# loehnea/bensolve

Measured on AMD Instinct MI355X. Metric: scalar LPs/sec (Benson phase 2, batched P2(v) solves incl. cut application), synthetic VLP q=5 n=500 m=1000, higher is better.
Workload: dtype f64

## Files before the change

### bensolve_amd/csrc/poly_engine.hip

```cpp
#include "common.h"
#include <vector>
#include <chrono>
#include <algorithm>
#include <cmath>
#include <thread>
#include <atomic>
#include <cstddef>

namespace bslv {

constexpr int MAXD = 16;
constexpr double POLY_EPS = 1e-9;
constexpr int PB = 256;
constexpr unsigned char F_USED = 1, F_IDEAL = 2, F_SLTN = 4;
constexpr int CRING = 1024;
constexpr int CSTRIDE = 8;
constexpr int LCAP = 16;
constexpr int LONGN = 64;
constexpr int ZMAX = 8;

struct Hp { double h[MAXD + 1]; };
struct Tri { int a, b, c; };

struct PolyView {
// ... 1965 lines not shown
        const int cv = __shfl(first, src, WAVE);
        const int *cL = D.fpool + D.foff[cj];
        const int cnj = D.flen[cj];
        const int *pool = P.pool + P.inc_off[cv];
        const int npool = P.inc_len[cv];
        bool found = false;
        for (int base = 0; base < npool; base += WAVE) {
            int k = base + lane;
            bool hit = false;
            if (k < npool) {
                int w = pool[k];
                if (w != fi && w != cj && D.flive[w] && D.flen[w] >= cn)
                    hit = isect3_count(A, ni, cL, cnj, D.fpool + D.foff[w], D.flen[w]) == cn;
            }
            if (__ballot(hit)) { found = true; break; }
        }
        if (lane == src) adj = !found;
    }
    Tri t{adj ? 1 : 0, 0, 0};
    pflag[(size_t)blockIdx.x * PB + threadIdx.x] = adj ? 1 : 0;
    Tri tot;
    (void)block_exscan(t, &tot, lds);
    if (threadIdx.x == 0) bsum[blockIdx.x] = tot;
}


__global__ __launch_bounds__(PB) void k_live_ranks(PolyView P, int nv, unsigned char *live)
{
    const int i = blockIdx.x * (PB / WAVE) + (threadIdx.x >> 6), lane = threadIdx.x & 63;
    if (i >= nv || !(P.flag[i] & F_USED)) return;
    const int *L = P.pool + P.inc_off[i];
    const int n = P.inc_len[i];
    for (int j = lane; j < n; j += WAVE) live[L[j]] = 1;
}
__global__ void k_bench_fill(PolyView P, int nv, unsigned long long seed)
{
    int i = blockIdx.x * blockDim.x + threadIdx.x;
    if (i >= nv) return;
    for (int k = 0; k < P.d; k++) {
        unsigned long long z = seed + 0x9E3779B97F4A7C15ull * ((unsigned long long)i * P.d + k + 1);
        z = (z ^ (z >> 30)) * 0xBF58476D1CE4E5B9ull;
        z = (z ^ (z >> 27)) * 0x94D049BB133111EBull;
        z ^= z >> 31;
        P.X[(size_t)k * P.cap + i] = (double)(z >> 11) * (1.0 / 9007199254740992.0) * 2.0 - 1.0;
    }
    P.flag[i] = F_USED;
    P.inc_len[i] = 0;
    P.inc_off[i] = 0;
}
#include "poly_rounds_kernels.inc"
#include "poly_rounds2_kernels.inc"
__device__ void k2v2_check_members(const K2V2 &V, int vs, const int *s_mem, int nm, const int *members, int nzero)
{
    RState *st = const_cast<RState *>(V.st);
    for (int m = threadIdx.x; m < nm; m += blockDim.x)
        for (int m2 = m + 1; m2 < nm; m2++)
            if (s_mem[m] == s_mem[m2] && atomicCAS(&st->err, 0, 4) == 0) {
                int c1 = -1, c2 = -1;
                for (int c = 0; c < nzero; c++) if (members[c] == s_mem[m]) { if (c1 < 0) c1 = c; else c2 = c; }
                st->err_info[0] = vs; st->err_info[1] = m; st->err_info[2] = m2; st->err_info[3] = s_mem[m]; st->err_info[4] = c1; st->err_info[5] = c2; st->err_info[6] = nzero;
            }
}
__device__ __forceinline__ int k2v2_round(const RState *st) { return st->round; }
__device__ __forceinline__ int k2v2_rank_base(const RState *st) { return st->rank_base; }
__device__ __forceinline__ void k2v2_sizes(const RState *st, int &S, int &go, int &nzero, int &nv0, int &ncross)
{
    S = st->S; go = st->go && !r2_halted(st); nzero = st->nzero; nv0 = st->nv; ncross = st->ncross;
}


}

using namespace bslv;

struct RoundsBuf;
struct Rounds2Buf;
struct bslv_poly {
    RoundsBuf *rounds = nullptr;
    Rounds2Buf *rounds2 = nullptr;
    bool rounds2_enabled = true;
    bool r2_spec = true;
    long r2_spec_void = 0;
    bool r2_mis = true;
    int chunk_cuts = 1024;
    int r2_defer = 0;
    bool r2_deferred = false;
    long r2_deferred_cuts = 0, r2_doomed = 0;
    bool r2_defer_mark = !(getenv("BSLV_DEFER_MARK") && atoi(getenv("BSLV_DEFER_MARK")) == 0);
    bool snap = false;
    unsigned long long *snapped_d = nullptr;
    int r2_min_cuts = 0;
    long r2_rounds = 0, r2_cuts = 0, r2_fallback_prunes = 0, r2_declined = 0, r2_chunks = 0, shuffle_seq = 0, r2_late_left = 0, r2_torn_reads = 0;
    long r2_fb_reason[5] = {0, 0, 0, 0, 0}, r2_fb_nm[20] = {0};
    int batch_mode = 1;
    long rounds_run = 0, conf_pairs = 0, conf_cuts = 0;
    int dense_streak = 0, dense_skip = 0;
    int d = 0, v2h = 0;
    std::vector<double> c;
    hipStream_t stream = nullptr;
    PolyView P{};
    int nv = 0;
    unsigned poolcap = 0, poolused = 0;
    int2 *E[2] = {nullptr, nullptr};
    int ecap = 0, ne = 0, ecur = 0;
    unsigned char *eflag = nullptr;
    int *ecount = nullptr; int ecountcap = 0;
    int *EP[2] = {nullptr, nullptr};
    bool hot = false, hot_enabled = true;
    struct EdgeSet { int2 *E[2] = {nullptr, nullptr}; int *EP[2] = {nullptr, nullptr}; unsigned char *eflag = nullptr; int ecap = 0, ne = 0, ecur = 0; } full, hotbuf;
    unsigned char *alive = nullptr; int alivecap = 0;
    int *hv_d = nullptr; int hvcap = 0;
    int *lslot_d = nullptr; int lslotcap = 0;
    unsigned *lbits_d = nullptr; size_t lbitscap = 0; int *lnslots_d = nullptr;
    long hot_chunks = 0, hot_elems = 0, hot_edges = 0;
    long n_spec = 0, n_declined = 0, n_k2_fallback = 0, n_single = 0;
    double tm_hot_begin = 0, tm_seq = 0, tm_hot_end = 0, tm_add_cuts = 0; long tm_seq_cuts = 0;
    double tm_realloc = 0; long n_realloc = 0;
    double tm_prep = 0, tm_classify_wait = 0, tm_newdual = 0;
    double tm_launch[4] = {0, 0, 0, 0};
    int *members = nullptr;
    Tri *bsum = nullptr; int bsumcap = 0;
    Tri *bsum2 = nullptr; size_t bsum2cap = 0;
    int *fm_cnt = nullptr, *fm_list = nullptr; size_t fmcap = 0, fmlistcap = 0; int fm_min = 4096; long n_fm = 0; bool member_lists = true;
    int largest_facet = 0;
    bool k2_noflags = getenv("BSLV_K2_NOFLAGS") != nullptr; long n_noflag_prunes = 0;
    long long window_blocks = 0x7FFFFFF0ll, win_max_blocks = 0; long n_win_prunes = 0, n_windows = 0;
    int shard_min = 32768; long n_sharded = 0; int2 *shard_e = nullptr; size_t shardcap = 0;
    int *nzlist = nullptr; size_t nzcap = 0;
    Tri *totals = nullptr;
    int *counters = nullptr;
    Tri *totals_h = nullptr; int *counters_h = nullptr;
    Mail *mail_h = nullptr, *mail_d = nullptr;
    Mail mail_v[4];
    long mail_torn_reads = 0;
    Mail *k2mail_d = nullptr;
    int *fstamp = nullptr, *flocal = nullptr, *nlocal = nullptr; int fcap = 0;
    unsigned long long *bits = nullptr; size_t bitscap = 0;
    int mailseq = 0;
    long cutseq = 0;
    size_t k2_lds = 0;
    int *ne_dev = nullptr;
    bool pend_k2 = false;
    int pend_seq = 0, pend_slot = 2, pend_ebase = 0, pend_nm = 0, pend_stamp = 0, pend_nzero = 0, pend_nv0 = 0, pend_ncross = 0; long long pend_len_ub = 0;
    int k2flip = 0;
    bool speculate = true;
    int cross_ub = CROSS_UB;
    CutDev *cutdev = nullptr;
    int *abort_d = nullptr;
    int *fcount = nullptr;
    int *zlist = nullptr, *zrows = nullptr;
    int pre_f = -1, pre_slot = 0, pre_nv = 0, pre_seq = 0;
    unsigned long long *k2dbg = nullptr;
    FILE *cutlog = nullptr;
    PairBlk *blks = nullptr; int blkcap = 0;
    unsigned char *pflag = nullptr; size_t pflagcap = 0;
    std::vector<double> Y, hp;
    std::vector<unsigned char> fapplied, fideal;
    std::vector<int> facet_of_rank;
    int nf = 0;
    bool initialised = false;
    std::vector<int> queue;
    std::vector<int> dual_edges;
    long pair_tests = 0, new_vertices = 0, cuts_applied = 0;
    double *hps_d = nullptr; int hpscap = 0; std::vector<double> hps_stage;
    unsigned long long *clsw = nullptr; size_t clswcap = 0;
    int *live_d = nullptr; int livecap = 0;
// ... 760 lines not shown
    for (int k = 0; k < d; k++)
        HIP_TRY(hipMemcpy(h->P.X + (size_t)k * h->P.cap, &soa[(size_t)k * n], n * sizeof(double), hipMemcpyHostToDevice));
    std::vector<unsigned char> fl(n, F_USED);
    for (int i = 1; i < n; i++) fl[i] |= F_IDEAL;
    HIP_TRY(hipMemcpy(h->P.flag, fl.data(), n, hipMemcpyHostToDevice));
    std::vector<unsigned> off(n);
    std::vector<int> len(n), pool;
    for (int i = 0; i < n; i++) { off[i] = (unsigned)pool.size(); len[i] = (int)inc[i].size(); pool.insert(pool.end(), inc[i].begin(), inc[i].end()); }
    HIP_TRY(hipMemcpy(h->P.inc_off, off.data(), n * sizeof(unsigned), hipMemcpyHostToDevice));
    HIP_TRY(hipMemcpy(h->P.inc_len, len.data(), n * sizeof(int), hipMemcpyHostToDevice));
    HIP_TRY(hipMemcpy(h->P.pool, pool.data(), pool.size() * sizeof(int), hipMemcpyHostToDevice));
    h->poolused = (unsigned)pool.size();
    std::vector<int2> E;
    for (int k = 0; k <= d; k++) for (int j = k + 1; j <= d; j++) E.push_back(int2{k, j});
    HIP_TRY(hipMemcpy(h->E[h->ecur], E.data(), E.size() * sizeof(int2), hipMemcpyHostToDevice));
    h->ne = (int)E.size();
    h->nv = n;
    h->facet_of_rank.resize(h->nf);
    for (int f = 0; f < h->nf; f++) h->facet_of_rank[f] = f;
    return 0;
}

static double gs_step(const double *x, double *H, double *R, int k, int n)
{
    double nrm_in = 0, scl = 0;
    for (int l = 0; l < n; l++) nrm_in += x[l] * x[l];
    nrm_in = std::sqrt(nrm_in);
    double *hr = H + (size_t)k * n;
    for (int l = 0; l < n; l++) hr[l] = x[l];
    for (int j = 0; j < k; j++) {
        double s = 0;
        for (int l = 0; l < n; l++) s += H[(size_t)j * n + l] * hr[l];
        for (int l = 0; l < n; l++) hr[l] -= s * H[(size_t)j * n + l];
    }
    for (int l = 0; l < n; l++) scl += hr[l] * hr[l];
    scl = std::sqrt(scl);
    if (scl < 1.0e-6) return 0;
    for (int l = 0; l < n; l++) hr[l] /= scl;
    for (int j = 0; j <= k; j++) {
        double s = 0;
        for (int l = 0; l < n; l++) s += H[(size_t)j * n + l] * x[l];
        R[k * (k + 1) / 2 + j] = s;
    }
    return scl / nrm_in;
}

extern "C" {

int bslv_poly_create(bslv_poly **out, int dim, int v2h, const double *c)
{
    if (!out || dim < 2 || dim > MAXD || v2h < 0 || v2h > 2) { set_error("bslv_poly_create: bad argument (2 <= dim <= %d)", MAXD); return BSLV_E_ARG; }
    if (bslv_device_count() < 1) { set_error("no HIP device available"); return BSLV_E_NODEVICE; }
    bslv_poly *h = new bslv_poly();
    h->d = dim; h->v2h = v2h;
    h->c.assign(dim, 0.0);
    if (c) h->c.assign(c, c + dim);
    h->P.d = dim;
    auto fail = [&](int code) { bslv_poly_destroy(h); return code; };
    if (hipStreamCreate(&h->stream) != hipSuccess) { set_error("hipStreamCreate failed"); return fail(BSLV_E_NODEVICE); }
    if (malloc0(&h->totals, 4 * sizeof(Tri)) != hipSuccess || malloc0(&h->counters, CRING * CSTRIDE * sizeof(int)) != hipSuccess || malloc0(&h->ne_dev, 4 * sizeof(int)) != hipSuccess || malloc0(&h->k2mail_d, 4 * sizeof(Mail)) != hipSuccess || hipMemset(h->k2mail_d, 0, 4 * sizeof(Mail)) != hipSuccess || malloc0(&h->cutdev, CRING * sizeof(CutDev)) != hipSuccess ||
        malloc0(&h->abort_d, 4 * sizeof(int)) != hipSuccess || hipMemset(h->abort_d, 0, 4 * sizeof(int)) != hipSuccess || malloc0(&h->zlist, CRING * ZMAX * sizeof(int)) != hipSuccess ||
        hipHostMalloc(&h->totals_h, 4 * sizeof(Tri)) != hipSuccess || hipHostMalloc(&h->counters_h, 4 * sizeof(int)) != hipSuccess ||
        hipHostMalloc(&h->mail_h, 4 * sizeof(Mail), hipHostMallocMapped | hipHostMallocCoherent) != hipSuccess ||
        hipHostGetDevicePointer((void **)&h->mail_d, h->mail_h, 0) != hipSuccess ||
        hipMemset(h->counters, 0, CRING * CSTRIDE * sizeof(int)) != hipSuccess) {
        set_error("allocation of scan scratch failed");
        return fail(BSLV_E_NOMEM);
    }
    memset((void *)h->mail_h, 0, 4 * sizeof(Mail));
    memset((void *)h->mail_v, 0, sizeof h->mail_v);
    for (int k = 0; k < 4; k++) h->mail_h[k].chk2 = mail_sum2(Tri{0, 0, 0}, 0);
    h->k2_lds = 128 * 1024;
    if (hipFuncSetAttribute((const void *)k2_fused_t<false>, hipFuncAttributeMaxDynamicSharedMemorySize, (int)h->k2_lds) != hipSuccess ||
        hipFuncSetAttribute((const void *)k2_fused_t<true>, hipFuncAttributeMaxDynamicSharedMemorySize, (int)h->k2_lds) != hipSuccess) {
        (void)hipGetLastError();
        h->k2_lds = 48 * 1024;
    }
    if (const char *cl = getenv("BSLV_CUT_LOG")) h->cutlog = fopen(cl, "w");
    if (getenv("BSLV_NO_SPEC")) h->speculate = false;
    if (getenv("BSLV_NO_HOT")) h->hot_enabled = false;
    if (getenv("BSLV_NO_ROUNDS2")) h->rounds2_enabled = false;
    if (const char *e = getenv("BSLV_R2_MIS")) h->r2_mis = atoi(e) != 0;
    if (const char *e = getenv("BSLV_R2_SPEC")) h->r2_spec = atoi(e) != 0;
    if (const char *e = getenv("BSLV_CHUNK_CUTS")) h->chunk_cuts = std::min(4096, std::max(32, atoi(e)));
    if (const char *e = getenv("BSLV_R2_MIN_CUTS")) h->r2_min_cuts = std::max(-1, atoi(e));
    if (const char *e = getenv("BSLV_POLY_SNAP")) h->snap = atoi(e) != 0;
    if (const char *e = getenv("BSLV_CROSS_UB")) h->cross_ub = std::max(0, atoi(e));
    if (const char *e = getenv("BSLV_K2_LDS")) h->k2_lds = (size_t)std::max(64, atoi(e));
    if (const char *e = getenv("BSLV_K2_WINDOW")) { const long long v = atoll(e); if (v > 0) h->window_blocks = std::min(v, PAIR_WINDOW_DEFAULT); }
    if (getenv("BSLV_K2_DEBUG") && malloc0(&h->k2dbg, 16 * sizeof(unsigned long long)) == hipSuccess) (void)hipMemset(h->k2dbg, 0, 16 * sizeof(unsigned long long));
    h->rounds = new RoundsBuf();
    std::vector<double> z(dim, 0.0);
    z[dim - 1] = -1.0;
    new_dual(h, z.data(), 1);
    *out = h;
    return 0;
}

void bslv_poly_destroy(bslv_poly *h)
{
    if (!h) return;
    if (getenv("BSLV_R2_REPORT") && h->r2_fallback_prunes) {
        fprintf(stderr, "r2: %ld prunes of rounds went through the multi-kernel path: %ld members > %d, %ld pair bitmap, %ld hash table, %ld bit matrix | members by power of two:", h->r2_fallback_prunes,
                h->r2_fb_reason[1], K2_MAXNM, h->r2_fb_reason[2], h->r2_fb_reason[3], h->r2_fb_reason[4]);
        for (int k = 0; k < 20; k++) if (h->r2_fb_nm[k]) fprintf(stderr, " 2^%d: %ld", k, h->r2_fb_nm[k]);
        fprintf(stderr, "\n");
    }
    if (getenv("BSLV_TIMING"))
        fprintf(stderr, "poly timing: add_cuts %.1f ms | hot_begin %.1f, sequences %.1f (%ld cuts, %.1f us each), hot_end %.1f ms | %ld hot chunks, %.0f elements, %.0f edges on average\n", h->tm_add_cuts,
                h->tm_hot_begin, h->tm_seq, h->tm_seq_cuts, h->tm_seq_cuts ? h->tm_seq * 1e3 / h->tm_seq_cuts : 0.0, h->tm_hot_end, h->hot_chunks,
                h->hot_chunks ? (double)h->hot_elems / h->hot_chunks : 0.0, h->hot_chunks ? (double)h->hot_edges / h->hot_chunks : 0.0),
        fprintf(stderr, "poly timing, per batch of cuts: dual slots %.2f ms, chunk preparation %.2f ms, waiting for the batched classification %.2f ms (totals); %ld re-allocations of element / edge / pool arrays, %.2f ms\n", h->tm_newdual, h->tm_prep, h->tm_classify_wait, h->n_realloc, h->tm_realloc),
        fprintf(stderr, "poly host per cut (us): queue round A %.1f, k_emit2 %.1f, round B in all %.1f, mailbox wait %.1f\n", h->tm_launch[0] / std::max(1L, h->n_single), h->tm_launch[1] / std::max(1L, h->n_single),
                h->tm_launch[2] / std::max(1L, h->n_single), h->tm_launch[3] / std::max(1L, h->n_single));
    if (h->cutlog) fclose(h->cutlog);
    if (h->k2dbg) {
        unsigned long long t[16];
        if (hipMemcpy(t, h->k2dbg, sizeof(t), hipMemcpyDeviceToHost) == hipSuccess && t[7])
            fprintf(stderr, "k2_fused phases (us/launch over %llu launches; rounds: per prune workgroup): P0a %.2f P0 %.2f P1 %.2f P2 %.2f P3 %.2f P4 %.2f P5 %.2f P6 %.2f | W %.1f nloc %.0f | members mean %.0f max %llu\n", t[7],
                    t[10] * 0.01 / t[7], t[0] * 0.01 / t[7], t[1] * 0.01 / t[7], t[2] * 0.01 / t[7], t[3] * 0.01 / t[7], t[4] * 0.01 / t[7], t[5] * 0.01 / t[7], t[6] * 0.01 / t[7], (double)t[8] / t[7], (double)t[9] / t[7],
                    (double)t[11] / t[7], t[12]);
        (void)hipFree(h->k2dbg);
    }
    auto fr = [](void *p) { if (p) (void)hipFree(p); };
    fr(h->P.X); fr(h->P.flag); fr(h->P.cls); fr(h->P.inc_off); fr(h->P.inc_len); fr(h->P.capx); fr(h->P.pool); fr(h->P.keep);
    fr(h->E[0]); fr(h->E[1]); fr(h->eflag); fr(h->members); fr(h->bsum); fr(h->bsum2); fr(h->fm_cnt); fr(h->fm_list); fr(h->nzlist); fr(h->totals); fr(h->counters); fr(h->ne_dev); fr(h->k2mail_d); fr(h->zlist); fr(h->zrows); fr(h->fcount); fr(h->cutdev); fr(h->abort_d);
    for (int k = 0; k < 2; k++) { fr(h->hotbuf.E[k]); fr(h->hotbuf.EP[k]); }
    fr(h->snapped_d);
    fr(h->hotbuf.eflag); fr(h->alive); fr(h->hv_d); fr(h->ecount); fr(h->lslot_d); fr(h->lbits_d); fr(h->lnslots_d);
    fr(h->shard_e); fr(h->blks); fr(h->pflag); fr(h->fstamp); fr(h->flocal); fr(h->nlocal); fr(h->bits); fr(h->hps_d); fr(h->clsw); fr(h->live_d); fr(h->anyminus); fr(h->idx_d); fr(h->val_d); fr(h->fl_d); fr(h->par_d); fr(h->r2f_d); fr(h->fhist_d); fr(h->chosen_d);
    if (h->rounds) { rounds_free(*h->rounds); delete h->rounds; }
    if (h->rounds2) { rounds2_free(*h->rounds2); delete h->rounds2; }
    if (h->totals_h) (void)hipHostFree(h->totals_h);
    if (h->counters_h) (void)hipHostFree(h->counters_h);
    if (h->mail_h) (void)hipHostFree((void *)h->mail_h);
    if (h->stream) (void)hipStreamDestroy(h->stream);
    delete h;
}

int bslv_poly_dual0_apex(bslv_poly *h)
{
    if (!h) return BSLV_E_ARG;
    h->fideal[0] = 0;
    h->Y[h->d - 1] = 0.0;
    v2h_map(h, h->Y.data(), 0, h->hp.data());
    return 0;
}

int bslv_poly_add(bslv_poly *h, const double *val, int ideal, int *rc_out)
{
    if (!h || !val || !rc_out) { set_error("bslv_poly_add: bad argument"); return BSLV_E_ARG; }
    int f = new_dual(h, val, ideal);
    if (!h->initialised) { h->queue.push_back(f); *rc_out = 0; return 0; }
    int rc = do_cut(h, f, rc_out);
    return rc ? rc : settle_k2(h);
}

int bslv_poly_init(bslv_poly *h, int *rc_out)
{
    if (!h || !rc_out) return BSLV_E_ARG;
    if (h->initialised) { set_error("bslv_poly_init: already initialised"); return BSLV_E_STATE; }
    const int d = h->d;
    int qn = (int)h->queue.size();
    if (qn < d) { *rc_out = 1; return 0; }
    std::vector<double> hpq((size_t)qn * (d + 1));
    for (int k = 0; k < qn; k++) memcpy(&hpq[(size_t)k * (d + 1)], &h->hp[(size_t)h->queue[k] * (d + 1)], (d + 1) * sizeof(double));
// ... 750 lines not shown
```

### bensolve_amd/csrc/poly_rounds2_host.inc

```
#include <string>
#include <deque>

struct Rounds2Buf {
    RState *st_d = nullptr;
    RState *mail_h = nullptr, *mail_d = nullptr;
    unsigned *alive = nullptr, *alive_prev = nullptr, *anym = nullptr, *bad = nullptr;
    int *selmap = nullptr, *sel = nullptr, *order = nullptr, *rcflag = nullptr;
    int bcap = 0;
    int *own = nullptr; int vcap = 0;
    unsigned long long *hw = nullptr; size_t hwcap = 0;
    int *cnt_g = nullptr, *nm_g = nullptr, *mem_g = nullptr; unsigned *adj_g = nullptr; int scap = 0;
    int *gout = nullptr, *gout_h = nullptr;
    int seq = 0;
    unsigned chunk_seed = 0;
    unsigned *M = nullptr, *selw = nullptr, *wm = nullptr; int *mcnt = nullptr; int wmcap = 0;
    int *fc2 = nullptr, *fl2 = nullptr, *fc_ticket = nullptr; int fc_slices = 0, fc_stride = 0;
};
constexpr int R2_ADJW = (K2_MAXNM * (K2_MAXNM - 1) / 2 + 31) / 32;
constexpr int R2_MAILS = 4;

static void rounds2_free(Rounds2Buf &V)
{
    auto fr = [](void *p) { if (p) (void)hipFree(p); };
    fr(V.st_d); fr(V.alive); fr(V.alive_prev); fr(V.anym); fr(V.bad); fr(V.selmap); fr(V.sel); fr(V.order); fr(V.rcflag); fr(V.own);
    fr(V.cnt_g); fr(V.nm_g); fr(V.mem_g); fr(V.adj_g); fr(V.gout); fr(V.hw); fr(V.M); fr(V.selw); fr(V.wm); fr(V.mcnt); fr(V.fc2); fr(V.fl2); fr(V.fc_ticket);
    if (V.mail_h) (void)hipHostFree(V.mail_h);
    if (V.gout_h) (void)hipHostFree(V.gout_h);
    V = Rounds2Buf();
}
static int rounds2_ensure(bslv_poly *h, Rounds2Buf &V, int Bc)
{
    hipStream_t s = h->stream;
    int rc;
    if (!V.st_d) {
        HIP_TRY(malloc0(&V.st_d, sizeof(RState)));
        HIP_TRY(hipHostMalloc(&V.mail_h, R2_MAILS * sizeof(RState), hipHostMallocMapped | hipHostMallocCoherent));
        HIP_TRY(hipHostGetDevicePointer((void **)&V.mail_d, V.mail_h, 0));
        memset(V.mail_h, 0, R2_MAILS * sizeof(RState));
        HIP_TRY(malloc0(&V.gout, 4 * sizeof(int)));
        HIP_TRY(hipHostMalloc(&V.gout_h, 4 * sizeof(int)));
        HIP_TRY(malloc0(&V.M, (size_t)R2_MAXC * (R2_MAXC / 32) * sizeof(unsigned)));
        HIP_TRY(malloc0(&V.selw, 64 * sizeof(unsigned)));
        HIP_TRY(malloc0(&V.mcnt, (size_t)R2_MAXC * sizeof(int)));
        if (hipFuncSetAttribute((const void *)k_r2_select3, hipFuncAttributeMaxDynamicSharedMemorySize, (int)((R2_MAXC / 32) * R2_MLD * sizeof(unsigned))) != hipSuccess ||
            hipFuncSetAttribute((const void *)k_r2_minit, hipFuncAttributeMaxDynamicSharedMemorySize, (int)(((size_t)R2_MAXC * (R2_MAXC / 32 + 1) + R2_MAXC + 64) * sizeof(unsigned))) != hipSuccess) {
            (void)hipGetLastError();
            h->r2_mis = false;
        }
    }
    if (h->P.cap > V.wmcap) { if ((rc = grow(&V.wm, (size_t)V.wmcap, (size_t)h->P.cap, s, true))) return rc; V.wmcap = h->P.cap; }
    if (Bc > V.bcap) {
        const int nc = std::max(Bc, 1024), nw = (nc + 31) / 32 + 2;
        if ((rc = grow(&V.alive, 0, (size_t)nw, s))) return rc;
        if ((rc = grow(&V.alive_prev, 0, (size_t)nw, s))) return rc;
        if ((rc = grow(&V.anym, 0, (size_t)nw, s))) return rc;
        if ((rc = grow(&V.bad, 0, (size_t)nw, s))) return rc;
        if ((rc = grow(&V.selmap, 0, (size_t)nc, s))) return rc;
        if ((rc = grow(&V.sel, 0, (size_t)nc, s))) return rc;
        if ((rc = grow(&V.order, 0, (size_t)nc, s))) return rc;
        if ((rc = grow(&V.rcflag, 0, (size_t)nc, s))) return rc;
        if ((rc = grow(&V.cnt_g, 0, (size_t)nc, s))) return rc;
        if ((rc = grow(&V.nm_g, 0, (size_t)nc, s))) return rc;
        if ((rc = grow(&V.mem_g, 0, (size_t)nc * K2_MAXNM, s))) return rc;
        if ((rc = grow(&V.adj_g, 0, (size_t)nc * R2_ADJW, s))) return rc;
        V.bcap = nc; V.scap = nc;
    }
    if (h->P.cap > V.vcap) { if ((rc = grow(&V.own, 0, (size_t)h->P.cap, s))) return rc; V.vcap = h->P.cap; }
    return 0;
}
template <class... A>
static void launch_r2_emit(int d, dim3 grid, hipStream_t s, A... a)
{
    switch (d) {
#define CASE(D) case D: hipLaunchKernelGGL(k_r2_emit<D>, grid, dim3(PB), 0, s, a...); break;
        CASE(2) CASE(3) CASE(4) CASE(5) CASE(6) CASE(7) CASE(8) CASE(9) CASE(10)
#undef CASE
    default: hipLaunchKernelGGL(k_r2_emit<0>, grid, dim3(PB), 0, s, a...); break;
    }
}
template <class... A>
static void launch_r2_classify3(int d, dim3 grid, hipStream_t s, A... a)
{
    switch (d) {
#define CASE(D) case D: hipLaunchKernelGGL(k_r2_classify3<D>, grid, dim3(PB), 0, s, a...); break;
        CASE(2) CASE(3) CASE(4) CASE(5) CASE(6) CASE(7) CASE(8) CASE(9) CASE(10)
#undef CASE
    default: hipLaunchKernelGGL(k_r2_classify3<0>, grid, dim3(PB), 0, s, a...); break;
    }
}
static inline bool rstate_try_read(const volatile RState *m, int seq, RState *out, long *torn)
{
    if (m->seq != seq) return false;
    __sync_synchronize();
    RState c;
    memcpy((void *)&c, (const void *)m, sizeof c);
    if (c.seq == seq) {
        const unsigned chk = c.chk;
        c.chk = 0; c.seq = 0;
        if (rstate_sum(c, seq) == chk) { c.chk = chk; c.seq = seq; *out = c; return true; }
    }
    if (torn) ++*torn;
    return false;
}
static int r2_wait(bslv_poly *h, Rounds2Buf &V, int seq, RState *out)
{
    volatile RState *m = V.mail_h + (seq % R2_MAILS);
    long torn = 0, drained = 0;
    for (long spin = 0; !rstate_try_read(m, seq, out, &torn); spin++) {
        if ((spin & 0xFFFF) == 0xFFFF) {
            hipError_t e = hipStreamQuery(h->stream);
            if (e == hipSuccess && ++drained > 1024) {
                set_error("poly engine: the round mailbox never reached a consistent state for seq %d (seq there: %d, %ld torn reads)", seq, (int)m->seq, torn);
                return BSLV_E_STATE;
            }
            if (e != hipSuccess && e != hipErrorNotReady) { set_error("poly engine: stream error %s", hipGetErrorString(e)); return BSLV_E_NODEVICE; }
        }
    }
    h->r2_torn_reads += torn;
    if (torn) { static const bool rep = getenv("BSLV_R2_REPORT") != nullptr; if (rep) fprintf(stderr, "r2: mailbox seq %d arrived before its state: %ld reads repeated\n", seq, torn); }
    return 0;
}

static int run_rounds2(bslv_poly *h, RoundsBuf &R, const std::vector<int> &todo, const std::vector<int> &fid_local, const std::vector<int> &rem, int *rc_out,
                       int Bc, int nw, std::vector<int> &left_out)
{
    left_out.clear();
    h->r2_deferred = false;
    if (!h->hot || h->pend_k2) { set_error("internal: run_rounds2 in the wrong state"); return BSLV_E_STATE; }
    if (!h->rounds2) h->rounds2 = new Rounds2Buf();
    Rounds2Buf &V = *h->rounds2;
    hipStream_t s = h->stream;
    const int d = h->d;
    int rc;
    if ((rc = rounds2_ensure(h, V, Bc))) return rc;
    if ((rc = rounds_ensure(h, R, Bc))) return rc;
    const int nw32 = (Bc + 31) / 32;
    const bool mis = h->r2_mis && Bc <= R2_MAXC;
    int nwp = 1;
    while (nwp < nw) nwp <<= 1;
    {
        std::vector<unsigned> alive(nw32 + 2, 0u);
        for (int k : todo) alive[k >> 5] |= 1u << (k & 31);
        HIP_TRY(hipMemcpyAsync(V.alive, alive.data(), (nw32 + 2) * sizeof(unsigned), hipMemcpyHostToDevice, s));
        HIP_TRY(hipMemsetAsync(V.anym, 0, (nw32 + 2) * sizeof(unsigned), s));
        HIP_TRY(hipMemsetAsync(V.bad, 0, (nw32 + 2) * sizeof(unsigned), s));
        HIP_TRY(hipMemsetAsync(V.rcflag, 0xFF, (size_t)Bc * sizeof(int), s));
        RState st0;
        memset(&st0, 0, sizeof st0);
        st0.nv = h->nv; st0.ne = h->ne; st0.nranks = (int)h->facet_of_rank.size(); st0.poolused = h->poolused;
        HIP_TRY(hipMemcpyAsync(V.st_d, &st0, sizeof st0, hipMemcpyHostToDevice, s));
        HIP_TRY(hipStreamSynchronize(s));
    }
    {
        const size_t need = (size_t)h->P.cap * nw;
        if (need > V.hwcap) { if ((rc = grow(&V.hw, 0, need, s))) return rc; V.hwcap = need; }
        const long long items = (long long)vm_count(h->P, h->nv) * nw;
        if (mis) {
            const int nel = vm_count(h->P, h->nv);
            if (nel > 0) hipLaunchKernelGGL(k_r2_words3, dim3((nel + PB - 1) / PB), dim3(PB), 0, s, h->P, (const unsigned long long *)h->clsw, nw, h->nv, V.hw, V.wm);
        } else if (items > 0) hipLaunchKernelGGL(k_r2_words, dim3((unsigned)((items + PB - 1) / PB)), dim3(PB), 0, s, h->P, (const unsigned long long *)h->clsw, nw, h->nv, V.hw);
        HIP_TRY(hipGetLastError());
    }
    if (mis) {
        HIP_TRY(hipMemsetAsync(V.M, 0, (size_t)Bc * nw * sizeof(unsigned), s));
        HIP_TRY(hipMemsetAsync(V.mcnt, 0, (size_t)Bc * sizeof(int), s));
    }
    const int rank0 = (int)h->facet_of_rank.size();
    {
        const int nranks = rank0 + Bc + 1;
        if (nranks > h->fcap) {
// ... 79 lines not shown
    int max_dv = 0, max_de = 0;
    bool stop_enq = false;
    auto clear_halt = [&]() -> int { HIP_TRY(hipMemsetAsync(&V.st_d->halt, 0, 2 * sizeof(int), s)); return 0; };
    auto drain = [&]() -> int {
        while (!inflight.empty()) {
            RState x;
            if ((rc = r2_wait(h, V, inflight.front().first, &x))) return rc;
            inflight.pop_front();
            h->r2_spec_void++;
        }
        cur = h->ecur;
        return 0;
    };
    auto launch_round = [&](bool ahead, int *seq_out, int *sub_out) -> int {
        const int nv = h->nv + (ahead ? gv : 0), ne = h->ne + (ahead ? ge : 0);
        const int nbv = (vm_count(h->P, std::min(nv, h->P.cap)) + PB - 1) / PB, nbe = std::max(1, (std::min(ne, h->ecap) + PB - 1) / PB);
        Tri *ebsum = h->bsum, *vbsum = h->bsum + nbe + 1;
        const int cslot = next_counter_slot(h);
        if (cslot < 0) { set_error("hipMemsetAsync failed"); return BSLV_E_NODEVICE; }
        int *counters = h->counters + CSTRIDE * cslot;
        const ZMarks Z{h->zlist + ZMAX * cslot, h->zrows, h->fcap, (int)h->cutseq};
        const int2 *Eold = h->E[cur];
        int2 *Enew = h->E[1 - cur];
        if (mis) {
            {
                const int items = ne + vm_count(h->P, std::min(nv, h->P.cap));
                static const int wgmax = getenv("BSLV_R2_MINIT_WG") ? std::max(1, atoi(getenv("BSLV_R2_MINIT_WG"))) : 256;
                const int nwg = std::max(1, std::min(wgmax, (items + 1023) / 1024));
                static const int probe_at = getenv("BSLV_R2_MINIT_PROBE") ? atoi(getenv("BSLV_R2_MINIT_PROBE")) : -1;
                static int probe_n = 0;
                static unsigned long long *probe_d = nullptr;
                unsigned long long *probe = nullptr;
                if (probe_at >= 0) {
                    if (!probe_d) (void)hipMalloc(&probe_d, 256 * 16 * sizeof(unsigned long long));
                    const int pos = (int)rounds + (int)inflight.size();
                    if (probe_n++ >= probe_at && pos == (getenv("BSLV_R2_MINIT_PROBE_POS") ? atoi(getenv("BSLV_R2_MINIT_PROBE_POS")) : 0) && probe_n < 1000000) {
                        probe = probe_d; probe_n = 1000000;
                        (void)hipMemsetAsync(probe_d, 0, 256 * 16 * sizeof(unsigned long long), s);
                    }
                }
                hipLaunchKernelGGL(k_r2_minit, dim3(nwg), dim3(1024), ((size_t)Bc * (nw + 1) + Bc + nw) * sizeof(unsigned), s, h->P, (const unsigned long long *)V.hw, (const unsigned *)V.wm, nw, Bc,
                                   (const RState *)V.st_d, Eold, (const unsigned *)V.alive, V.M, V.mcnt, (const int *)R.tc, V.st_d, std::min(ne, h->ecap), vm_count(h->P, std::min(nv, h->P.cap)), probe);
                if (probe) {
                    std::vector<unsigned long long> pr(256 * 16);
                    (void)hipStreamSynchronize(s);
                    (void)hipMemcpy(pr.data(), probe_d, pr.size() * 8, hipMemcpyDeviceToHost);
                    unsigned long long t0 = ~0ull, t4 = 0;
                    for (int g = 0; g < nwg; g++) { t0 = std::min(t0, pr[g * 16]); t4 = std::max(t4, pr[g * 16 + 4]); }
                    fprintf(stderr, "minit probe: nwg %d items %d (ne %d) Bc %d nw %d round %d, whole %.1f us\n", nwg, items, ne, Bc, nw, (int)rounds + (int)inflight.size(), (t4 - t0) / 100.0);
                    const char *nm[4] = {"zero", "items", "queue", "or"};
                    for (int k = 0; k < 4; k++) {
                        double mn = 1e30, mx = 0, sm = 0;
                        for (int g = 0; g < nwg; g++) { const double d = (pr[g * 16 + k + 1] - pr[g * 16 + k]) / 100.0; mn = std::min(mn, d); mx = std::max(mx, d); sm += d; }
                        fprintf(stderr, "  %-6s min %.1f mean %.1f max %.1f us\n", nm[k], mn, sm / nwg, mx);
                    }
                    double st_mn = 1e30, st_mx = 0, qs = 0, qmx = 0, nz = 0;
                    for (int g = 0; g < nwg; g++) { const double d = (pr[g * 16] - t0) / 100.0; st_mn = std::min(st_mn, d); st_mx = std::max(st_mx, d); qs += pr[g * 16 + 6]; qmx = std::max(qmx, (double)pr[g * 16 + 6]); nz += pr[g * 16 + 7]; }
                    { double a = 0, b2 = 0, c = 0, d2 = 0; for (int g = 0; g < nwg; g++) { a += pr[g * 16 + 8]; b2 += pr[g * 16 + 9]; c += pr[g * 16 + 10]; d2 = std::max(d2, (double)pr[g * 16 + 11]); }
                      fprintf(stderr, "  per wave (mean over %d waves): resolve + first fetch %.1f us, giving %.1f us, waiting for the next item's words %.1f us; slowest wave %.1f us\n", nwg * 16, a / nwg / 16 / 100, b2 / nwg / 16 / 100, c / nwg / 16 / 100, d2 / 100); }
                    fprintf(stderr, "  start skew max %.1f us; queue items mean %.0f max %.0f; non-zero words per wg %.0f\n", st_mx, qs / nwg, qmx, nz / nwg);
                }
            }
            hipLaunchKernelGGL(k_r2_select3, dim3(1), dim3(1024), (size_t)nw * R2_MLD * sizeof(unsigned), s, Bc, nw, V.alive, V.alive_prev, V.M, V.mcnt,
                               V.selmap, V.sel, V.order, V.rcflag, V.st_d, V.selw, depth);
            hipLaunchKernelGGL(k_r2_assign3, dim3(nbv), dim3(PB), 0, s, h->P, (const unsigned long long *)V.hw, (const unsigned *)V.wm, nw, (const RState *)V.st_d, (const unsigned *)V.selw,
                               (const int *)V.selmap, R.cutof, counters, h->zlist + ZMAX * cslot);
        } else {
            hipLaunchKernelGGL(k_r2_prep, dim3(nbe + nbv), dim3(PB), (size_t)(3 * nw + 2) * sizeof(unsigned), s, h->P, (const unsigned long long *)V.hw, nw,
                               (const RState *)V.st_d, Eold, nbe, (const unsigned *)V.alive, V.anym, V.bad, V.own, (const int *)R.tc, V.st_d);
            hipLaunchKernelGGL(k_r2_select, dim3(1), dim3(1024), 0, s, Bc, V.alive, V.alive_prev, V.anym, V.bad, V.selmap, V.sel, V.order, V.rcflag, V.st_d, depth);
            hipLaunchKernelGGL(k_r2_assign, dim3(nbv), dim3(PB), 0, s, h->P, (const unsigned long long *)V.hw, nw, (const RState *)V.st_d, (const int *)V.own,
                               (const int *)V.selmap, R.cutof, counters, h->zlist + ZMAX * cslot);
        }
        hipLaunchKernelGGL(k_flags2, dim3(nbe + nbv), dim3(PB), 0, s, h->P, Eold, ne, (const int *)&V.st_d->ne, nbe, nv, (const int *)counters, h->eflag, h->ecount, ebsum, vbsum, Z, (const int *)&V.st_d->nv,
                           (const int *)&V.st_d->halt, mis ? R2Own{(const int *)R.cutof, (const unsigned long long *)V.hw, (const unsigned *)V.wm, (const unsigned *)V.selw, (const int *)V.selmap, nw}
                                                           : R2Own{nullptr, nullptr, nullptr, nullptr, nullptr, 0});
        launch_r2_emit(d, dim3(nbe + nbv), s, h->P, (const double *)h->hps_d, (const int *)V.sel, R.cutof, Eold, nbe, (const unsigned char *)h->eflag, (const int *)h->ecount,
                       (const Tri *)ebsum, (const Tri *)vbsum, Enew, h->members, (const int *)counters, V.st_d, h->P.cap, h->ecap, h->poolcap,
                       (const int *)h->EP[cur], h->EP[1 - cur], Z, (const unsigned long long *)V.hw, (const unsigned *)V.wm, nw, (int *)nullptr,
                       (const unsigned *)V.selw, (const int *)V.selmap);
        const int S_ub = std::max(1, std::min(Bc - napplied - nredundant, V.scap));
        const K2V2 KV{V.st_d, R.cutof, V.mem_g, V.adj_g, V.cnt_g, V.nm_g, R2_ADJW, &V.st_d->pair_tests, V.fc2, V.fl2, V.fc_ticket, V.fc2 ? V.fc_slices : 0, V.fc_stride};
        const int seq = ++V.seq;
        const int want = std::max(2048, 2 * last_ncross);
        launch_r2_classify3(d, dim3(std::max(1, std::min(4096, (want + PB / nwp - 1) / (PB / nwp)))), s, h->P, (const double *)h->hps_d, Bc, nw, nwp, (const RState *)V.st_d,
                            (const unsigned *)V.alive, V.hw, V.wm, (int *)nullptr, mis ? 1 : 0);
        hipLaunchKernelGGL(k2_fused_t<true>, dim3(S_ub), dim3(K2T), h->k2_lds, s, h->P, h->members, 0, 0, 0, h->fcount, h->flocal, (int)(h->k2_lds / 8), Enew, 0,
                           (int *)nullptr, h->totals + 2, h->k2mail_d, 0, h->k2dbg, (const CutDev *)nullptr, h->abort_d, (int *)nullptr, Hp{}, (int *)nullptr,
                           (int *)nullptr, KV);
        hipLaunchKernelGGL(k_r2_k2emit, dim3(S_ub), dim3(K2T), 0, s, V.st_d, (const int *)V.cnt_g, (const int *)V.nm_g, (const unsigned *)V.adj_g, (const int *)V.mem_g,
                           R2_ADJW, Enew, h->EP[1 - cur], h->ecap, V.mail_d + (seq % R2_MAILS), seq, (const unsigned long long *)V.hw, (const unsigned *)V.wm, nw, (const unsigned *)V.alive);
        HIP_TRY(hipGetLastError());
        cur = 1 - cur;
        *seq_out = seq; *sub_out = S_ub;
        return 0;
    };
    auto prepare = [&](bool ahead) -> int {
        const int nv = h->nv + (ahead ? gv : 0), ne = h->ne + (ahead ? ge : 0);
        const int nbv = (vm_count(h->P, std::min(nv, h->P.cap)) + PB - 1) / PB, nbe = std::max(1, (std::min(ne, h->ecap) + PB - 1) / PB);
        const size_t pool_need = (size_t)h->poolused + (size_t)(ahead ? 4 : 1) * 65536;
        if (ahead) {
            if (nbe + nbv + 2 > h->bsumcap || pool_need > h->poolcap || h->ecap > h->ecountcap) return -1;
            return 0;
        }
        if ((rc = ensure_pool(h, pool_need + (depth ? 8 * 65536 : 0)))) return rc;
        if (h->ecap > h->ecountcap) { if ((rc = grow(&h->ecount, 0, (size_t)h->ecap, s))) return rc; h->ecountcap = h->ecap; }
        const int nbv2 = (vm_count(h->P, std::min(h->nv + 2 * gv, h->P.cap)) + PB - 1) / PB, nbe2 = std::max(1, (std::min(h->ne + 2 * ge, h->ecap) + PB - 1) / PB);
        if ((rc = ensure_bsum(h, std::max(nbe + nbv, depth ? nbe2 + nbv2 : 0) + 2))) return rc;
        return 0;
    };
    for (;;) {
        while (!stop_enq && (int)inflight.size() <= depth) {
            const bool ahead = !inflight.empty();
            const int pr = prepare(ahead);
            if (pr < 0) break;
            if (pr > 0) return pr;
            int sq = 0, sub = 0;
            if ((rc = launch_round(ahead, &sq, &sub))) return rc;
            inflight.emplace_back(sq, sub);
        }
        if (inflight.empty()) break;
        int seq = inflight.front().first;
        const int S_ub = inflight.front().second;
        inflight.pop_front();
        const int nv = h->nv, ne = h->ne;
        RState m;
        if ((rc = r2_wait(h, V, seq, &m))) return rc;
        if (m.halt == 2) {
            if ((rc = drain())) return rc;
            HIP_TRY(hipMemsetAsync(V.anym, 0, (nw32 + 2) * sizeof(unsigned), s));
            HIP_TRY(hipMemsetAsync(V.bad, 0, (nw32 + 2) * sizeof(unsigned), s));
            if (mis) {
                HIP_TRY(hipMemsetAsync(V.M, 0, (size_t)Bc * nw * sizeof(unsigned), s));
                HIP_TRY(hipMemsetAsync(V.mcnt, 0, (size_t)Bc * sizeof(int), s));
            }
            if ((rc = clear_halt())) return rc;
            gv *= 4; ge *= 4;
            h->r2_spec_void++;
            continue;
        }
        if (dbg) fprintf(stderr, "r2 round %d: S %d alive %d redundant %d | go %d declined %d nminus %d nzero %d nsurv %d ncross %d pairs %d eover %d k2abort %d | nv %d ne %d pool %u\n",
                         m.round, m.S, m.nalive, m.nredundant, m.go, m.declined, m.nminus, m.nzero, m.nsurv, m.ncross, m.epairs, m.eover, m.k2abort, m.nv, m.ne, m.poolused);
        if (m.err && getenv("BSLV_R2_DEBUG")) {
            for (int which = 0; which < 2; which++) {
                const int el = m.err_info[1 + which], k = m.err_info[4];
                unsigned char fl = 0; int tcv = -7, ownv = -7; unsigned long long wm = 0, we = 0; signed char cl = 0; int co = -7;
                (void)hipMemcpy(&fl, h->P.flag + el, 1, hipMemcpyDeviceToHost);
                (void)hipMemcpy(&tcv, R.tc + el, 4, hipMemcpyDeviceToHost);
                (void)hipMemcpy(&ownv, V.own + el, 4, hipMemcpyDeviceToHost);
                (void)hipMemcpy(&co, R.cutof + el, 4, hipMemcpyDeviceToHost);
                (void)hipMemcpy(&cl, h->P.cls + el, 1, hipMemcpyDeviceToHost);
                (void)hipMemcpy(&wm, h->clsw + (size_t)(k >> 5) * h->P.cap + el, 8, hipMemcpyDeviceToHost);
                (void)hipMemcpy(&we, V.hw + (size_t)el * nw + (k >> 5), 8, hipMemcpyDeviceToHost);
                std::vector<double> hp(d + 3), x(d);
                (void)hipMemcpy(hp.data(), h->hps_d + (size_t)k * (d + 3), (d + 3) * 8, hipMemcpyDeviceToHost);
                for (int c = 0; c < d; c++) (void)hipMemcpy(&x[c], h->P.X + (size_t)c * h->P.cap + el, 8, hipMemcpyDeviceToHost);
                double sdot = 0; for (int c = 0; c < d; c++) sdot = fma(hp[c], x[c], sdot);
                int hvpos = -1;
                { std::vector<int> hv(h->P.nhv); if (h->P.nhv) (void)hipMemcpy(hv.data(), h->hv_d, (size_t)h->P.nhv * 4, hipMemcpyDeviceToHost); for (int t = 0; t < h->P.nhv; t++) if (hv[t] == el) hvpos = t; }
                fprintf(stderr, "r2 debug: element %d flag %d tc %d own %d cutof %d cls %d | class of cut %d: word-major %d, element-major %d | s %.17g alpha %.17g hi %.17g lo %.17g | position in hot list %d (nhv %d, nv_base %d, nv %d, cap %d)\n",
                        el, fl, tcv, ownv, co, cl, k, (int)((wm >> (2 * (k & 31))) & 3), (int)((we >> (2 * (k & 31))) & 3), sdot, hp[d], hp[d + 1], hp[d + 2], hvpos, h->P.nhv, h->P.nv_base, h->nv, h->P.cap);
            }
        }
        if (m.err == 4) {
            {
                const int el = m.err_info[3];
                std::vector<int> hv(std::max(h->P.nhv, 1));
                if (h->P.nhv) (void)hipMemcpy(hv.data(), h->hv_d, (size_t)h->P.nhv * 4, hipMemcpyDeviceToHost);
                int dups = 0, nondec = 0;
// ... 161 lines not shown
```

### bensolve_amd/csrc/poly_rounds2_kernels.inc

```

struct RState {
    int nv, ne, nranks;
    unsigned poolused;
    int round, S, rank_base, napplied, nredundant, nalive, stuck;
    int go, declined, nminus, nzero, zero_ub, nsurv, ncross, newlen;
    int nv_next, ne_next; unsigned pool_next, pool_e, pool_z;
    int epairs, eover, k2abort;
    long long pair_tests;
    int halt;
    int halt2;
    int err, err_info[7];
    double err_d[12];
    unsigned chk;
    int seq;
};
static_assert(offsetof(RState, halt2) == offsetof(RState, halt) + sizeof(int), "k_flags2 reads (halt, halt2) as two consecutive ints");
__host__ __device__ __forceinline__ unsigned rstate_sum(const RState &s, int seq)
{
    const unsigned *w = reinterpret_cast<const unsigned *>(&s);
    unsigned c = 0x9E3779B9u;
    for (unsigned i = 0; i < sizeof(RState) / 4; i++) c = c * 31u + w[i];
    return c + (unsigned)seq * 2654435761u;
}
__device__ __forceinline__ void rstate_publish(RState *st, RState *mail, int seq)
// ... 782 lines not shown
        if (P.flag[i] & F_USED) {
            c = 1;
            unsigned m = st->S > 0 ? wm[i] : 0u;
            int nown = 0, ofirst = -1, ominus = -1;
            while (m) {
                const int w = __ffs((int)m) - 1;
                m &= m - 1;
                if (!selw[w]) continue;
                const unsigned long long word = words[(size_t)i * nw + w];
                const unsigned t = r2_touch32(word) & selw[w];
                if (!t) continue;
                const unsigned mn = r2_minus32(word) & selw[w];
                if (mn) ominus = w * 32 + __ffs((int)mn) - 1;
                if (ofirst < 0) ofirst = w * 32 + __ffs((int)t) - 1;
                nown += __popc(t);
            }
            if (ominus >= 0) { c = -1; s = selmap[ominus]; isminus = 1; }
            else if (nown > 0) {
                c = 0; iszero = 1;
                s = nown == 1 ? selmap[ofirst] : -1 - nown;
                zlen = zero_room(P, i, nown);
                if (nown == 1 && P.inc_len[i] > LONGN) { const int k = atomicAdd(&counters[3], 1); if (k < ZMAX) zlist[k] = i; }
            }
        }
        P.cls[i] = c;
        cutof[i] = s;
    }
    const unsigned long long bm = __ballot(isminus), bz = __ballot(iszero);
    if (bz) {
#pragma unroll
        for (int o = 32; o > 0; o >>= 1) zlen += __shfl_xor(zlen, o, WAVE);
    }
    if ((threadIdx.x & 63) == 0) {
        if (bm) atomicAdd(&counters[0], __popcll(bm));
        if (bz) { atomicAdd(&counters[1], __popcll(bz)); atomicAdd(&counters[2], zlen); }
    }
}
template <int D>
__device__ __forceinline__ void r2_classify3_body(const PolyView &P, const double *__restrict__ hps, int B, int nw, int nwp, const RState *st, const unsigned *__restrict__ alive,
                                                  unsigned long long *__restrict__ hw, unsigned *__restrict__ wm, int *mcnt, int block, int nblocks, int nthr, int packed = 1)
{
    if (!st->go || r2_halted(st)) return;
    const int vpb = nthr / nwp, w = threadIdx.x & (nwp - 1), lv = threadIdx.x / nwp, lane = threadIdx.x & 63;
    const int ncross = st->ncross, first = st->nv_next - ncross;
    const int d = D > 0 ? D : P.d;
    const unsigned aw = w < nw ? alive[w] : 0u;
    for (int base = block * vpb; base < ncross; base += nblocks * vpb) {
        const bool act = base + lv < ncross;
        const int i = first + base + lv;
        unsigned touch = 0u;
        if (act && aw) {
            double x[D > 0 ? D : MAXD];
#pragma unroll
            for (int k = 0; k < (D > 0 ? D : MAXD); k++) x[k] = k < d ? P.X[(size_t)k * P.cap + i] : 0.0;
            const bool ideal = P.flag[i] & F_IDEAL;
            const int bend = min(32, B - w * 32);
            unsigned plus = 0, notminus = 0;
            for (int bb = 0; bb < bend; bb++) {
                const double *h = hps + (size_t)(w * 32 + bb) * (d + 3);
                double s = 0.0;
#pragma unroll
                for (int k = 0; k < (D > 0 ? D : MAXD); k++) if (k < d) s = fma(h[k], x[k], s);
                const double hi = ideal ? 0.0 + POLY_EPS : h[d + 1], lo = ideal ? 0.0 - POLY_EPS : h[d + 2];
                plus |= (unsigned)(s > hi) << bb;
                notminus |= (unsigned)(s > lo) << bb;
            }
            const unsigned valid = bend == 32 ? 0xFFFFFFFFu : ((1u << bend) - 1u);
            const unsigned lowb = (plus | ~notminus) & valid, highb = notminus & valid;
            hw[(size_t)i * nw + w] = packed ? (unsigned long long)(lowb ^ highb) | ((unsigned long long)(lowb & ~highb) << 32) : spread32(lowb) | (spread32(highb) << 1);
            touch = (lowb ^ highb) & aw;
            unsigned mi = mcnt ? (lowb & ~highb & aw) : 0u;
            while (mi) { const int b = __ffs((int)mi) - 1; mi &= mi - 1; atomicAdd(&mcnt[w * 32 + b], 1); }
        }
        const unsigned long long bt = __ballot(touch != 0u);
        if (act && w == 0) wm[i] = (unsigned)((bt >> (lane & ~(nwp - 1))) & (nwp == 32 ? 0xFFFFFFFFull : ((1ull << nwp) - 1ull)));
    }
}
template <int D>
__global__ __launch_bounds__(PB) void k_r2_classify3(PolyView P, const double *__restrict__ hps, int B, int nw, int nwp, const RState *st, const unsigned *__restrict__ alive,
                                                     unsigned long long *__restrict__ hw, unsigned *__restrict__ wm, int *mcnt, int packed)
{
    r2_classify3_body<D>(P, hps, B, nw, nwp, st, alive, hw, wm, mcnt, (int)blockIdx.x, (int)gridDim.x, PB, packed);
}

__global__ __launch_bounds__(PB) void k_r2_mark_doomed(PolyView P, const unsigned long long *__restrict__ hw, const unsigned *__restrict__ wm, int nw, int nv,
                                                       const unsigned *__restrict__ alive, int *count)
{
    const int idx = blockIdx.x * PB + threadIdx.x;
    if (idx >= vm_count(P, nv)) return;
    const int i = vm_id(P, idx);
    const unsigned char fl = P.flag[i];
    if (!(fl & F_USED) || (fl & F_SLTN)) return;
    unsigned m = wm ? wm[i] : 0xFFFFFFFFu;
    bool doomed = false;
    for (int w = 0; w < nw && !doomed; w++) {
        if (!((m >> w) & 1u) || alive[w] == 0u) continue;
        const unsigned long long word = hw[(size_t)i * nw + w];
        doomed = ((wm ? r2_minus32(word) : compress32(word & ~(word >> 1))) & alive[w]) != 0u;
    }
    if (doomed) { P.flag[i] = fl | F_SLTN; atomicAdd(count, 1); }
}

__global__ __launch_bounds__(PB) void k_r2_words(PolyView P, const unsigned long long *__restrict__ words, int nw, int nv, unsigned long long *__restrict__ hw)
{
    const long long t = (long long)blockIdx.x * PB + threadIdx.x;
    const int w = (int)(t % nw);
    const long long idx = t / nw;
    if (idx >= vm_count(P, nv)) return;
    const int i = vm_id(P, (int)idx);
    hw[(size_t)i * nw + w] = words[(size_t)w * P.cap + i];
}

__global__ __launch_bounds__(K2T) void k_r2_k2emit(RState *st, const int *__restrict__ cnt_g, const int *__restrict__ nm_g, const unsigned *__restrict__ adj_g,
                                                   const int *__restrict__ mem_g, int adjw_cap, int2 *E, int *EP, int ecap, RState *mail, int seq,
                                                   const unsigned long long *__restrict__ hw, const unsigned *__restrict__ wm, int nw, const unsigned *__restrict__ alive_g)
{
    __shared__ Tri lds[16];
    __shared__ int s_carry;
    (void)hw; (void)wm; (void)nw; (void)alive_g;
    const int S = st->S, s = blockIdx.x, tid = threadIdx.x;
    const int h2 = st->halt2;
    if (S <= 0 || !st->go || st->halt || (h2 != 0 && h2 != seq)) {
        if (s == 0 && tid == 0) rstate_publish(st, mail, seq);
        return;
    }
    Tri part{0, 0, 0};
    for (int k = tid; k < S; k += K2T) { const int c = cnt_g[k]; if (c > 0) { part.b += c; if (k < s) part.a += c; } if (c < 0) part.c += 1; }
    part = block_sum(part, lds);
    const int ebase = st->ne_next, before = part.a, total = part.b;
    const bool over = (long long)ebase + total > ecap;
    if (s == 0 && tid == 0) {
        st->epairs = total; st->eover = over; st->k2abort = part.c;
        if (over || part.c > 0) st->halt2 = seq;
        if (!over) { st->nv = st->nv_next; st->ne = ebase + total; st->poolused = st->pool_next; }
        rstate_publish(st, mail, seq);
    }
    if (over || s >= S) return;
    const int cnt = cnt_g[s];
    if (cnt <= 0) return;
    const int nm = nm_g[s];
    const int nadjw = (int)(((long long)nm * (nm - 1) / 2 + 31) / 32);
    const unsigned *adj = adj_g + (size_t)s * adjw_cap;
    const int *mem = mem_g + (size_t)s * K2_MAXNM;
    if (tid == 0) s_carry = 0;
    __syncthreads();
    for (int w0 = 0; w0 < nadjw; w0 += K2T) {
        const int ww = w0 + tid;
        unsigned word = ww < nadjw ? adj[ww] : 0u;
        Tri t{(int)__popc(word), 0, 0};
        Tri tot;
        const Tri ex = block_exscan(t, &tot, lds);
        int at = ebase + before + s_carry + ex.a;
        while (word) {
            const int bbit = __ffs((int)word) - 1;
            word &= word - 1;
            int i, j;
            pair_decode32(ww * 32 + bbit, nm, i, j);
            E[at] = int2{mem[i], mem[j]};
            if (EP) EP[at] = -1;
            at++;
        }
        __syncthreads();
        if (tid == 0) s_carry += tot.a;
        __syncthreads();
    }
}
// ... 63 lines not shown
```

Baseline: 168,700.

## Add cut-per-lane classify kernel keeping cut hyperplanes in registers

Adds a new rounds2 classify kernel in which each lane owns one cut and holds its hyperplane coefficients in registers. Vertices are streamed through LDS in groups of V, and wave ballots produce the packed plus/minus words directly. It is used by default when the MIS path is active and nw<=32, replacing the vertex-parallel classify3 launch. The aim is to stop reloading cut data for every vertex and to get the bit words from ballots instead of per-thread loops. The cost is high register pressure (4*DM doubles per lane), a fixed grid size, and a serial per-vertex loop inside each block.

```diff
diff --git a/bensolve_amd/csrc/poly_engine.hip b/bensolve_amd/csrc/poly_engine.hip
--- a/bensolve_amd/csrc/poly_engine.hip
+++ b/bensolve_amd/csrc/poly_engine.hip
@@ -2071,6 +2071,8 @@
     bool r2_spec = true;
     long r2_spec_void = 0;
     bool r2_mis = true;
+    bool r2_cls_cutlane = true;
+    int r2_cls_v = 8, r2_cls_grid = 512;
     int chunk_cuts = 1024;
     int r2_defer = 0;
     bool r2_deferred = false;
@@ -2997,6 +2999,9 @@
     if (getenv("BSLV_NO_ROUNDS2")) h->rounds2_enabled = false;
     if (const char *e = getenv("BSLV_R2_MIS")) h->r2_mis = atoi(e) != 0;
     if (const char *e = getenv("BSLV_R2_SPEC")) h->r2_spec = atoi(e) != 0;
+    if (const char *e = getenv("BSLV_R2_CLS")) h->r2_cls_cutlane = atoi(e) != 0;
+    if (const char *e = getenv("BSLV_R2_CLS_V")) h->r2_cls_v = std::min(R2_CLVMAX, std::max(1, atoi(e)));
+    if (const char *e = getenv("BSLV_R2_CLS_GRID")) h->r2_cls_grid = std::min(4096, std::max(1, atoi(e)));
     if (const char *e = getenv("BSLV_CHUNK_CUTS")) h->chunk_cuts = std::min(4096, std::max(32, atoi(e)));
     if (const char *e = getenv("BSLV_R2_MIN_CUTS")) h->r2_min_cuts = std::max(-1, atoi(e));
     if (const char *e = getenv("BSLV_POLY_SNAP")) h->snap = atoi(e) != 0;
diff --git a/bensolve_amd/csrc/poly_rounds2_host.inc b/bensolve_amd/csrc/poly_rounds2_host.inc
--- a/bensolve_amd/csrc/poly_rounds2_host.inc
+++ b/bensolve_amd/csrc/poly_rounds2_host.inc
@@ -86,6 +86,16 @@
         CASE(2) CASE(3) CASE(4) CASE(5) CASE(6) CASE(7) CASE(8) CASE(9) CASE(10)
 #undef CASE
     default: hipLaunchKernelGGL(k_r2_classify3<0>, grid, dim3(PB), 0, s, a...); break;
+    }
+}
+template <class... A>
+static void launch_r2_classify_cl(int d, dim3 grid, hipStream_t s, A... a)
+{
+    switch (d) {
+#define CASE(D) case D: hipLaunchKernelGGL(k_r2_classify_cl<D>, grid, dim3(PB), 0, s, a...); break;
+        CASE(2) CASE(3) CASE(4) CASE(5) CASE(6) CASE(7) CASE(8) CASE(9) CASE(10)
+#undef CASE
+    default: hipLaunchKernelGGL(k_r2_classify_cl<0>, grid, dim3(PB), 0, s, a...); break;
     }
 }
 static inline bool rstate_try_read(const volatile RState *m, int seq, RState *out, long *torn)
@@ -331,9 +341,13 @@
         const int S_ub = std::max(1, std::min(Bc - napplied - nredundant, V.scap));
         const K2V2 KV{V.st_d, R.cutof, V.mem_g, V.adj_g, V.cnt_g, V.nm_g, R2_ADJW, &V.st_d->pair_tests, V.fc2, V.fl2, V.fc_ticket, V.fc2 ? V.fc_slices : 0, V.fc_stride};
         const int seq = ++V.seq;
-        const int want = std::max(2048, 2 * last_ncross);
-        launch_r2_classify3(d, dim3(std::max(1, std::min(4096, (want + PB / nwp - 1) / (PB / nwp)))), s, h->P, (const double *)h->hps_d, Bc, nw, nwp, (const RState *)V.st_d,
-                            (const unsigned *)V.alive, V.hw, V.wm, (int *)nullptr, mis ? 1 : 0);
+        if (mis && nw <= 32 && h->r2_cls_cutlane)
+            launch_r2_classify_cl(d, dim3(h->r2_cls_grid), s, h->P, (const double *)h->hps_d, Bc, nw, h->r2_cls_v, (const RState *)V.st_d, (const unsigned *)V.alive, V.hw, V.wm, (int *)nullptr);
+        else {
+            const int want = std::max(2048, 2 * last_ncross);
+            launch_r2_classify3(d, dim3(std::max(1, std::min(4096, (want + PB / nwp - 1) / (PB / nwp)))), s, h->P, (const double *)h->hps_d, Bc, nw, nwp, (const RState *)V.st_d,
+                                (const unsigned *)V.alive, V.hw, V.wm, (int *)nullptr, mis ? 1 : 0);
+        }
         hipLaunchKernelGGL(k2_fused_t<true>, dim3(S_ub), dim3(K2T), h->k2_lds, s, h->P, h->members, 0, 0, 0, h->fcount, h->flocal, (int)(h->k2_lds / 8), Enew, 0,
                            (int *)nullptr, h->totals + 2, h->k2mail_d, 0, h->k2dbg, (const CutDev *)nullptr, h->abort_d, (int *)nullptr, Hp{}, (int *)nullptr,
                            (int *)nullptr, KV);
diff --git a/bensolve_amd/csrc/poly_rounds2_kernels.inc b/bensolve_amd/csrc/poly_rounds2_kernels.inc
--- a/bensolve_amd/csrc/poly_rounds2_kernels.inc
+++ b/bensolve_amd/csrc/poly_rounds2_kernels.inc
@@ -888,6 +888,80 @@
 {
     r2_classify3_body<D>(P, hps, B, nw, nwp, st, alive, hw, wm, mcnt, (int)blockIdx.x, (int)gridDim.x, PB, packed);
 }
+constexpr int R2_CLVMAX = 32;
+constexpr int R2_CLG = 4;
+static_assert((PB / 64) * R2_CLG * 64 >= R2_MAXC, "the waves of a workgroup hold every cut of a chunk in their registers");
+template <int D>
+__global__ __launch_bounds__(PB) void k_r2_classify_cl(PolyView P, const double *__restrict__ hps, int B, int nw, int V, const RState *st, const unsigned *__restrict__ alive,
+                                                       unsigned long long *__restrict__ hw, unsigned *__restrict__ wm, int *mcnt)
+{
+    constexpr int DM = D > 0 ? D : MAXD;
+    __shared__ double xs[DM * R2_CLVMAX];
+    __shared__ unsigned ideal_s[R2_CLVMAX], touch_s[R2_CLVMAX];
+    if (!st->go || r2_halted(st)) return;
+    const int ncross = st->ncross, first = st->nv_next - ncross;
+    if ((int)blockIdx.x * V >= ncross) return;
+    const int d = D > 0 ? D : P.d;
+    const int lane = threadIdx.x & 63, half = lane >> 5, wave = __builtin_amdgcn_readfirstlane((int)(threadIdx.x >> 6)), ng = (nw + 1) / 2;
+    double hn[R2_CLG][DM], hhi[R2_CLG], hlo[R2_CLG];
+    unsigned aw0[R2_CLG], aw1[R2_CLG];
+    unsigned long long vmask[R2_CLG];
+    int mc[R2_CLG];
+#pragma unroll
+    for (int j = 0; j < R2_CLG; j++) {
+        const int g = wave + j * (PB / 64), cut = g * 64 + lane;
+        aw0[j] = g < ng ? alive[2 * g] : 0u;
+        aw1[j] = (g < ng && 2 * g + 1 < nw) ? alive[2 * g + 1] : 0u;
+        const int nvalid = max(0, min(64, B - g * 64));
+        vmask[j] = nvalid == 64 ? ~0ull : ((1ull << nvalid) - 1ull);
+        const bool ld = (aw0[j] | aw1[j]) != 0u && cut < B;
+        const double *h = hps + (size_t)(ld ? cut : 0) * (d + 3);
+#pragma unroll
+        for (int k = 0; k < DM; k++) hn[j][k] = (ld && k < d) ? h[k] : 0.0;
+        hhi[j] = ld ? h[d + 1] : 0.0;
+        hlo[j] = ld ? h[d + 2] : 0.0;
+        mc[j] = 0;
+    }
+    for (int base = blockIdx.x * V; base < ncross; base += gridDim.x * V) {
+        const int nvs = min(V, ncross - base);
+        for (int t = threadIdx.x; t < d * nvs; t += PB) { const int k = t / nvs, v = t - k * nvs; xs[k * R2_CLVMAX + v] = P.X[(size_t)k * P.cap + first + base + v]; }
+        if ((int)threadIdx.x < nvs) { ideal_s[threadIdx.x] = P.flag[first + base + threadIdx.x] & F_IDEAL; touch_s[threadIdx.x] = 0u; }
+        __syncthreads();
+        for (int v = 0; v < nvs; v++) {
+            const int i = first + base + v;
+            double x[DM];
+#pragma unroll
+            for (int k = 0; k < DM; k++) x[k] = k < d ? xs[k * R2_CLVMAX + v] : 0.0;
+            const bool ideal = ideal_s[v] != 0u;
+            unsigned tb = 0u;
+#pragma unroll
+            for (int j = 0; j < R2_CLG; j++) {
+                if ((aw0[j] | aw1[j]) == 0u) continue;
+                const int g = wave + j * (PB / 64);
+                double s = 0.0;
+#pragma unroll
+                for (int k = 0; k < DM; k++) if (k < d) s = fma(hn[j][k], x[k], s);
+                const double hi = ideal ? 0.0 + POLY_EPS : hhi[j], lo = ideal ? 0.0 - POLY_EPS : hlo[j];
+                const unsigned long long plus = __ballot(s > hi), notminus = __ballot(s > lo);
+                const unsigned long long low64 = (plus | ~notminus) & vmask[j], high64 = notminus & vmask[j];
+                const unsigned long long t64 = low64 ^ high64, m64 = low64 & ~high64;
+                const unsigned awh = half ? aw1[j] : aw0[j];
+                if ((lane & 31) == 0 && awh)
+                    hw[(size_t)i * nw + 2 * g + half] = (unsigned long long)(unsigned)(t64 >> (32 * half)) | ((unsigned long long)(unsigned)(m64 >> (32 * half)) << 32);
+                if ((unsigned)t64 & aw0[j]) tb |= 1u << (2 * g);
+                if ((unsigned)(t64 >> 32) & aw1[j]) tb |= 2u << (2 * g);
+                if (mcnt) mc[j] += (int)((m64 >> lane) & 1ull) & (int)((awh >> (lane & 31)) & 1u);
+            }
+            if (lane == 0 && tb) atomicOr(&touch_s[v], tb);
+        }
+        __syncthreads();
+        if ((int)threadIdx.x < nvs) wm[first + base + threadIdx.x] = touch_s[threadIdx.x];
+    }
+    if (mcnt) {
+#pragma unroll
+        for (int j = 0; j < R2_CLG; j++) if (mc[j]) atomicAdd(&mcnt[(wave + j * (PB / 64)) * 64 + lane], mc[j]);
+    }
+}
 
 __global__ __launch_bounds__(PB) void k_r2_mark_doomed(PolyView P, const unsigned long long *__restrict__ hw, const unsigned *__restrict__ wm, int nw, int nv,
                                                        const unsigned *__restrict__ alive, int *count)
```

Measured after the change: 171,300 (median of 6 runs). 1.5% higher.
